# Dylan-H-Wang/skin-sm3

Measured on AMD Instinct MI355X. Metric: SM3 pretrain images/sec (paired 224x224), higher is better.
Workload: dtype bf16

## Files before the change

### skin-sm3_amd/csrc/conv_igemm.hip

```cpp
#include <stdlib.h>

#include <atomic>
#include <type_traits>

#include "conv_common.h"

using namespace sm3conv;


namespace {

#ifdef SM3_STAMP
__device__ unsigned long long* g_stamp_buf = nullptr;
__device__ long g_stamp_cap = 0;
struct StampRec {
    unsigned long long t_entry, r_entry, t_loop0 = 0, t_loop1 = 0, seg[4] = {0, 0, 0, 0}, mark[8] = {0, 0, 0, 0, 0, 0, 0, 0};
    int nsteps = 0;
    __device__ StampRec() : t_entry(__builtin_amdgcn_s_memtime()), r_entry(__builtin_amdgcn_s_memrealtime()) {}
    __device__ ~StampRec() {
        const unsigned long long t_exit = __builtin_amdgcn_s_memtime();
        const long wave = ((long)blockIdx.y * gridDim.x + blockIdx.x) * (blockDim.x / 64) + (threadIdx.x >> 6);
        if ((threadIdx.x & 63) == 0 && g_stamp_buf && wave < g_stamp_cap) {
            unsigned long long* o = g_stamp_buf + wave * 24;
            o[0] = t_entry; o[1] = t_loop0; o[2] = t_loop1; o[3] = t_exit;
            o[4] = seg[0]; o[5] = seg[1]; o[6] = seg[2]; o[7] = seg[3];
            o[8] = (unsigned long long)nsteps; o[9] = blockIdx.x; o[10] = r_entry; o[11] = __builtin_amdgcn_s_memrealtime();
            for (int i = 0; i < 8; ++i) o[12 + i] = mark[i];
            o[20] = threadIdx.x >> 6;
        }
    }
};
#define SM3_STAMP_NOW() __builtin_amdgcn_s_memtime()
#define SM3_MARK(i) (stamp.mark[i] = __builtin_amdgcn_s_memtime())
#else
#define SM3_MARK(i) ((void)0)
#endif

constexpr int kVarPw = 2, kVarNoX = 4, kVarHalo = 16, kVarGrp = 64;
template <typename T, int BM, int BN, int WM, int WN, int STAGES, int EPI, bool SEG = false, int VAR = 0>
__global__ __launch_bounds__(WM* WN * 64, (EPI >= 1 && STAGES == 1) ? 4 : 2) void conv_igemm_kernel(const ConvParams p) {
    static_assert(STAGES == 1 || STAGES == 4, "one-stage loop, or the 4-stage ring of the small-grid launches");
    constexpr bool PW = (VAR & kVarPw) != 0, NOX = (VAR & kVarNoX) != 0;
    constexpr bool HALO = (VAR & kVarHalo) != 0;
    constexpr bool GRP = (VAR & kVarGrp) != 0;
    static_assert(!GRP || (EPI == 0 && !SEG && VAR == kVarGrp), "kVarGrp: the general epilogue, one K segment");
    static_assert(!HALO || (EPI >= 1 && STAGES == 1 && !SEG && !(VAR & kVarPw) && sizeof(T) == 2 && WM * WN == 4),
                  "kVarHalo: 16-bit lean one-stage kernels, 4 waves");
    static_assert(!NOX || EPI == 3, "kVarNoX: the fused BN-backward epilogue");
#ifdef SM3_STAMP
    StampRec stamp;
#endif
    constexpr bool LEAN = EPI >= 1;
    static_assert(!(SEG && EPI == 1) && !(SEG && STAGES > 2), "segments: data-gradient epilogues, 1 or 2 stages");
    constexpr int NT = WM * WN * 64;
    constexpr int RPP = NT / 8;
    constexpr int AI = BM / RPP, BI = BN / RPP;
    constexpr int WTM = BM / WM, WTN = BN / WN, TM = WTM / 32, TN = WTN / 32;
    constexpr int SZ = sizeof(T);
    constexpr int A_BYTES = BM * 128, B_BYTES = BN * 128, STAGE = A_BYTES + B_BYTES;
    constexpr int LEAN_PITCH = BN * 2 + 16;
    constexpr int CP = BN + 4;
    constexpr int C_BYTES = LEAN ? BM * LEAN_PITCH : WTM * CP * 4;
    constexpr int MAIN_BYTES = (STAGES * STAGE > C_BYTES) ? STAGES * STAGE : C_BYTES;
    static_assert(AI >= 1 && BI >= 1 && TM >= 1 && TN >= 1, "tile too small");

    extern __shared__ __attribute__((aligned(16))) char smem[];

    const int wave = __builtin_amdgcn_readfirstlane((int)threadIdx.x >> 6);
    const int tid = (int)threadIdx.x, lane = tid & 63;
    const int wm = wave / WN, wn = wave % WN;

    int bid = blockIdx.x;
    {
        const int nwg = gridDim.x, q = nwg >> 3, r = nwg & 7, xcd = bid & 7, slot = bid >> 3;
        bid = (xcd < r ? xcd * (q + 1) : r * (q + 1) + (xcd - r) * q) + slot;
    }
    const int bn = bid % p.tilesN, bm = bid / p.tilesN;
    const int m0 = bm * BM, n0 = bn * BN;

    const long grp = GRP ? (long)blockIdx.y : 0;
    const char* const gx = GRP ? p.x + grp * p.g_x_bytes : p.x;
    const char* const gw = GRP ? p.w + grp * p.g_w_bytes : p.w;
    char* const gy = GRP ? p.y + grp * p.g_y_bytes : p.y;
    float* const gpart = (GRP && p.partials) ? p.partials + grp * p.Co : p.partials;
    const long part_ld = GRP ? (long)p.part_ld : (long)p.Co;
    const __amdgpu_buffer_rsrc_t rx = __builtin_amdgcn_make_buffer_rsrc((void*)gx, 0, p.x_bytes, 0x00020000);
    const __amdgpu_buffer_rsrc_t rw = __builtin_amdgcn_make_buffer_rsrc((void*)gw, 0, p.w_bytes, 0x00020000);
    const __amdgpu_buffer_rsrc_t rx1 =
        SEG ? __builtin_amdgcn_make_buffer_rsrc((void*)p.x1, 0, p.x1_bytes, 0x00020000) : rx;
    const __amdgpu_buffer_rsrc_t rw1 =
        SEG ? __builtin_amdgcn_make_buffer_rsrc((void*)p.w1, 0, p.w1_bytes, 0x00020000) : rw;
    const int tile_view = (p.fz_view_tiles > 0 && bm >= p.fz_view_tiles) ? 1 : 0;

    const int pos = tid & 7;
    int a_pix[AI], a_iy0[AI], a_ix0[AI];
    uint32_t a_ch[AI], a_off[AI], b_off[BI];
    uint32_t b_off1[SEG ? BI : 1];
#pragma unroll
    for (int i = 0; i < AI; ++i) {
        const int r = (tid >> 3) + i * RPP;
        a_ch[i] = (uint32_t)((pos ^ (r >> 1)) & 7) * 16u;
        const int m = m0 + r;
        if constexpr (HALO) {
            a_iy0[i] = a_ix0[i] = a_pix[i] = 0;
            continue;
        }
        if constexpr (PW) {
            a_iy0[i] = a_ix0[i] = 0;
            a_pix[i] = m < p.M ? m : -1;
            continue;
        }
        if (m < p.M) {
            const int n = fdiv(m, p.div_HoWo);
            const int rem = m - n * p.HoWo;
            const int oy = fdiv(rem, p.div_Wo);
            const int ox = rem - oy * p.Wo;
            a_iy0[i] = oy * p.sy;
            a_ix0[i] = ox * p.sx;
            a_pix[i] = (n * p.Hi + a_iy0[i]) * p.Wi + a_ix0[i];
        } else {
            a_iy0[i] = -(1 << 20);
            a_ix0[i] = 0;
            a_pix[i] = 0;
        }
    }
#pragma unroll
    for (int i = 0; i < BI; ++i) {
        const int r = (tid >> 3) + i * RPP;
        const int co = n0 + r;
        b_off[i] = (co < p.Co) ? (uint32_t)co * (uint32_t)(p.w_row_stride * SZ) + (uint32_t)((pos ^ (r >> 1)) & 7) * 16u
                               : kOOB;
        if constexpr (SEG) {
            if (co < p.Co) b_off[i] += (uint32_t)tile_view * p.w_view_bytes;
            b_off1[i] = (co < p.Co) ? (uint32_t)co * (uint32_t)(p.w1_row_stride * SZ) + (uint32_t)((pos ^ (r >> 1)) & 7) * 16u +
                                          (uint32_t)tile_view * p.w1_view_bytes
                                    : kOOB;
        }
    }
    const uint32_t row_bytes = (uint32_t)p.Ci * SZ;
    const uint32_t row_bytes1 = SEG ? (uint32_t)p.Ci1 * SZ : row_bytes;
    int cur_src = 0;

    auto set_tap = [&](int t) {
        if constexpr (SEG) cur_src = __builtin_amdgcn_readfirstlane((int)p.tap_src[t]);
        const uint32_t rb = (SEG && cur_src) ? row_bytes1 : row_bytes;
        if constexpr (PW) {
#pragma unroll
            for (int i = 0; i < AI; ++i) a_off[i] = a_pix[i] >= 0 ? (uint32_t)a_pix[i] * rb + a_ch[i] : kOOB;
            return;
        }
        const int ddy = p.dy[t], ddx = p.dx[t];
        const int dpix = ddy * p.Wi + ddx;
#pragma unroll
        for (int i = 0; i < AI; ++i) {
            const int iy = a_iy0[i] + ddy, ix = a_ix0[i] + ddx;
            const bool ok = ((unsigned)iy < (unsigned)p.Hi) && ((unsigned)ix < (unsigned)p.Wi);
            a_off[i] = ok ? (uint32_t)(a_pix[i] + dpix) * rb + a_ch[i] : kOOB;
        }
    };
    const uint32_t smem_lds = (uint32_t)(uintptr_t)((__attribute__((address_space(3))) char*)smem);
    auto dma_stage = [&](int stage, uint32_t soff_a, uint32_t soff_b) {
        const uint32_t sA = smem_lds + (uint32_t)(stage * STAGE + wave * (8 * 128));
        const uint32_t sB = sA + A_BYTES;
        if (SEG && cur_src) {
#pragma unroll
            for (int i = 0; i < AI; ++i) dma16(rx1, sA + i * (RPP * 128), a_off[i], soff_a);
#pragma unroll
            for (int i = 0; i < BI; ++i) dma16(rw1, sB + i * (RPP * 128), b_off1[SEG ? i : 0], soff_b);
            return;
        }
#pragma unroll
        for (int i = 0; i < AI; ++i) dma16(rx, sA + i * (RPP * 128), a_off[i], soff_a);
#pragma unroll
        for (int i = 0; i < BI; ++i) dma16(rw, sB + i * (RPP * 128), b_off[i], soff_b);
    };

    f32x16 acc[TM][TN];
#pragma unroll
    for (int i = 0; i < TM; ++i)
#pragma unroll
        for (int j = 0; j < TN; ++j)
#pragma unroll
            for (int r = 0; r < 16; ++r) acc[i][j][r] = 0.f;

    const int frow = lane & 31, fh = lane >> 5;
    uint32_t fa_base[TM], fb_base[TN];
#pragma unroll
    for (int i = 0; i < TM; ++i) fa_base[i] = lds_off(wm * WTM + i * 32 + frow, fh);
#pragma unroll
    for (int j = 0; j < TN; ++j) fb_base[j] = A_BYTES + lds_off(wn * WTN + j * 32 + frow, fh);

// ... 68 lines not shown
                const int n = fdiv(m, p.div_HoWo);
                const int rem = m - n * p.HoWo;
                const int oy = fdiv(rem, p.div_Wo);
                const int ox = rem - oy * p.Wo;
                const unsigned ym = (oy > 0 ? 1u : 0u) | 2u | (oy + 1 < p.Hi ? 4u : 0u);
                const unsigned xm = (ox > 0 ? 1u : 0u) | 2u | (ox + 1 < p.Wi ? 4u : 0u);
                tap_ok[i] = ((ym & 1u) ? xm : 0u) | ((ym & 2u) ? xm << 3 : 0u) | ((ym & 4u) ? xm << 6 : 0u);
            }
        }
        uint32_t fbh[TN];
#pragma unroll
        for (int j = 0; j < TN; ++j) fbh[j] = (uint32_t)p.halo_a_bytes + lds_off(wn * WTN + j * 32 + frow, fh);
        const int kchunks = p.kchunks;
#ifdef SM3_STAMP
        stamp.mark[1] = stamp.t_loop0 = SM3_STAMP_NOW();
        stamp.nsteps = 9 * kchunks;
#endif
#pragma unroll 1
        for (int c = 0; c < kchunks; ++c) {
#pragma unroll 1
            for (int tt = 0; tt < 9; ++tt) {
#ifdef SM3_STAMP
                const unsigned long long q0 = SM3_STAMP_NOW();
#endif
                if ((c | tt) != 0) __syncthreads();
#ifdef SM3_STAMP
                const unsigned long long q1 = SM3_STAMP_NOW();
#endif
                if (tt == 0) halo_issue((uint32_t)c * 128u);
                const uint32_t soff_b = (uint32_t)p.wtap[tt] * row_bytes + (uint32_t)c * 128u;
#pragma unroll
                for (int i = 0; i < BI; ++i) dma16(rw, sBw + i * (RPP * 128), b_off[i], soff_b);
                const int ddy = p.dy[tt], ddx = p.dx[tt];
                const int bit = (ddy + 1) * 3 + ddx + 1, shift = hoff + ddy * p.Wi + ddx;
                uint32_t fah[TM];
#pragma unroll
                for (int i = 0; i < TM; ++i) {
                    const uint32_t own = lds_off(frag_row[i] + shift, fh);
                    fah[i] = ((tap_ok[i] >> bit) & 1u) ? own : (uint32_t)HR * 128u + (own & 255u);
                }
#ifdef SM3_STAMP
                const unsigned long long q2 = SM3_STAMP_NOW();
#endif
                dma_drain();
#ifdef SM3_STAMP
                const unsigned long long q3 = SM3_STAMP_NOW();
#endif
                __syncthreads();
#ifdef SM3_STAMP
                const unsigned long long q4 = SM3_STAMP_NOW();
#endif
#pragma unroll
                for (int kk = 0; kk < 4; ++kk) {
                    uint4 fa[TM], fb[TN];
#pragma unroll
                    for (int i = 0; i < TM; ++i) fa[i] = *reinterpret_cast<const uint4*>(smem + (fah[i] ^ (kk << 5)));
#pragma unroll
                    for (int j = 0; j < TN; ++j) fb[j] = *reinterpret_cast<const uint4*>(smem + (fbh[j] ^ (kk << 5)));
#pragma unroll
                    for (int i = 0; i < TM; ++i)
#pragma unroll
                        for (int j = 0; j < TN; ++j) mma_frag<T>(fa[i], fb[j], acc[i][j]);
                }
#ifdef SM3_STAMP
                const unsigned long long q5 = SM3_STAMP_NOW();
                stamp.seg[0] += q2 - q1; stamp.seg[1] += q5 - q4; stamp.seg[2] += q3 - q2; stamp.seg[3] += (q1 - q0) + (q4 - q3);
#endif
            }
        }
#ifdef SM3_STAMP
        stamp.t_loop1 = SM3_STAMP_NOW();
#endif
        __syncthreads();
    } else {
    dma_stage(0, 0, wtap_off);
    if constexpr (STAGES > 2) {
        constexpr int PER = AI + BI;
        for (int s = 1; s < STAGES - 1 && s < nsteps; ++s) {
            advance();
            dma_stage(s, (uint32_t)kc * 128u, wtap_off + (uint32_t)kc * 128u);
        }
        for (int s = 0; s < nsteps; ++s) {
            const int younger = min(STAGES - 2, nsteps - 1 - s);
            if (younger >= 2) asm volatile("s_waitcnt vmcnt(%0)" ::"n"(2 * PER) : "memory");
            else if (younger == 1) asm volatile("s_waitcnt vmcnt(%0)" ::"n"(PER) : "memory");
            else dma_drain();
            __syncthreads();
            if (s + STAGES - 1 < nsteps) {
                advance();
                dma_stage((s + STAGES - 1) % STAGES, (uint32_t)kc * 128u, wtap_off + (uint32_t)kc * 128u);
            }
            compute(s % STAGES);
        }
        __syncthreads();
    } else {
        dma_drain();
        __syncthreads();
        SM3_MARK(1);
#ifdef SM3_STAMP
        stamp.nsteps = nsteps;
#endif
        for (int s = 0; s < nsteps; ++s) {
#ifdef SM3_STAMP
            const unsigned long long q0 = SM3_STAMP_NOW();
#endif
            compute(0);
#ifdef SM3_STAMP
            const unsigned long long q1 = SM3_STAMP_NOW();
#endif
            __syncthreads();
#ifdef SM3_STAMP
            const unsigned long long q2 = SM3_STAMP_NOW();
            stamp.seg[1] += q1 - q0; stamp.seg[3] += q2 - q1;
#endif
            if (s + 1 < nsteps) {
                advance();
                dma_stage(0, (uint32_t)kc * 128u, wtap_off + (uint32_t)kc * 128u);
#ifdef SM3_STAMP
                const unsigned long long q3 = SM3_STAMP_NOW();
#endif
                dma_drain();
#ifdef SM3_STAMP
                const unsigned long long q4 = SM3_STAMP_NOW();
#endif
                __syncthreads();
#ifdef SM3_STAMP
                const unsigned long long q5 = SM3_STAMP_NOW();
                stamp.seg[0] += q3 - q2; stamp.seg[2] += q4 - q3; stamp.seg[3] += q5 - q4;
#endif
            }
        }
#ifdef SM3_STAMP
        stamp.t_loop0 = stamp.mark[1];
        stamp.t_loop1 = SM3_STAMP_NOW();
#endif
    }
    }
    SM3_MARK(2);

    if constexpr (LEAN) {
        static_assert(sizeof(T) == 2, "lean epilogue is for the 16-bit types");
        constexpr int CPR = BN / 8, RSTEP = NT / CPR, NPASS = BM / RSTEP;
        char* sC = smem;
        float* sStat = reinterpret_cast<float*>(smem + (HALO ? p.halo_stat_off : MAIN_BYTES));
        const uint32_t ones = ones2<T>();
        const int cc = tid % CPR, r0 = tid / CPR;
        const int ncol = n0 + cc * 8;
        const bool fz = EPI == 3 && p.fz_partials != nullptr;
        const bool fzx = !NOX && fz && p.fz_x != nullptr;
        uint32_t eoff[EPI >= 2 ? NPASS : 1];
        uint4 pre_add[EPI >= 2 ? NPASS : 1], pre_x[(EPI == 3 && !NOX) ? NPASS : 1];
        unsigned pre_mk[EPI == 3 ? NPASS : 1];
        constexpr int NEARLY = (EPI == 3 && !NOX) ? NPASS / 2 : NPASS;
        const bool dense_out = PW || (p.osy == 1 && p.osx == 1 && p.ooy == 0 && p.oox == 0 && p.HWout == p.HoWo);
        const uint32_t pw_base = (uint32_t)(((long)(m0 + r0) * p.Co + ncol) * 2), pw_step = (uint32_t)RSTEP * (uint32_t)p.Co * 2u;
        auto request = [&](int k) {
            const int m = m0 + r0 + k * RSTEP;
            eoff[k] = ~0u;
            pre_add[k] = make_uint4(0, 0, 0, 0);
            if constexpr (EPI == 3) {
                if constexpr (!NOX) pre_x[k] = make_uint4(0, 0, 0, 0);
                pre_mk[k] = 0xffu;
            }
            if constexpr (PW) {
                if (m < p.M && ncol < p.Co) {
                    eoff[k] = pw_base + (uint32_t)k * pw_step;
                    if (p.addend) pre_add[k] = ldg16<true>(p.addend + eoff[k]);
                    if constexpr (EPI == 3) {
                        if constexpr (!NOX) {
                            if (fzx) pre_x[k] = ldg16<true>(p.fz_x + eoff[k]);
                        }
                        if (fz && p.fz_mask) pre_mk[k] = p.fz_mask[eoff[k] >> 4];
                    }
                }
                return;
            }
            if (m < p.M && ncol < p.Co) {
                long opix = m;
                int nn = 0, oy = 0, ox = 0;
                if (!dense_out || p.add_sp_h) {
                    nn = fdiv(m, p.div_HoWo);
                    const int rem = m - nn * p.HoWo;
                    oy = fdiv(rem, p.div_Wo);
                    ox = rem - oy * p.Wo;
                    if (!dense_out) opix = (long)nn * p.HWout + (long)(oy * p.osy + p.ooy) * p.Wout + (ox * p.osx + p.oox);
                }
                eoff[k] = (uint32_t)((opix * p.Co + ncol) * 2);
                if (p.addend) {
                    if (p.add_sp_h && !dense_out) {
                        pre_add[k] = ldg16<true>(p.addend + ((long)m * p.Co + ncol) * 2);
                    } else if (p.add_sp_h) {
                        if (((oy | ox) & 1) == 0)
                            pre_add[k] = ldg16<true>(p.addend + ((((long)nn * p.add_sp_h + (oy >> 1)) * p.add_sp_w + (ox >> 1)) * p.Co + ncol) * 2);
                    } else {
                        pre_add[k] = ldg16<true>(p.addend + eoff[k]);
                    }
                }
                if constexpr (EPI == 3) {
                    if constexpr (!NOX) {
                        if (fzx) pre_x[k] = ldg16<true>(p.fz_x + eoff[k]);
                    }
                    if (fz && p.fz_mask) pre_mk[k] = p.fz_mask[eoff[k] >> 4];
                }
            }
        };
        const bool epl = p.ep_scale != nullptr || p.ep_rv != nullptr;
        const bool aff = epl || (SEG && p.col_bias);
        constexpr int NCB = TN, CBW = 32;
        const int lcol = frow;
        float esc_j[NCB], esh_j[NCB];
#pragma unroll
        for (int j = 0; j < NCB; ++j) {
            esc_j[j] = 1.f;
            esh_j[j] = 0.f;
            const int gcol = n0 + wn * WTN + j * CBW + lcol;
            if (epl && gcol < p.Co) {
                if (p.ep_rv) {
                    ep_affine(p, gcol, esc_j[j], esh_j[j]);
                } else {
                    esc_j[j] = p.ep_scale[tile_view * p.Co + gcol];
                    esh_j[j] = p.ep_shift[tile_view * p.Co + gcol];
                }
            }
            if constexpr (SEG) {
                if (p.col_bias && gcol < p.Co) esh_j[j] += p.col_bias[tile_view * p.Co + gcol];
            }
        }
        if constexpr (EPI >= 2) {
#pragma unroll
            for (int k = 0; k < NEARLY; ++k) request(k);
        }
        SM3_MARK(6);
        const bool early_relu = epl && p.ep_relu && (EPI == 1 || !p.addend) && !p.ep_mask;
        auto stage_tile = [&](auto stats_c, auto aff_c, auto relu_c) {
            constexpr bool STATS = decltype(stats_c)::value, AFF = decltype(aff_c)::value, RELU = decltype(relu_c)::value;
#pragma unroll
            for (int j = 0; j < TN; ++j) {
                float s1 = 0.f, s2 = 0.f;
                char* colp = sC + (wn * WTN + j * 32 + frow) * 2 + (wm * WTM + 4 * fh) * LEAN_PITCH;
                const uint32_t colp_lds = (uint32_t)(uintptr_t)((__attribute__((address_space(3))) char*)colp);
                const float esc = esc_j[j], esh = esh_j[j];
#pragma unroll
                for (int i = 0; i < TM; ++i)
#pragma unroll
                    for (int q = 0; q < 8; ++q) {
                        float v0 = acc[i][j][2 * q], v1 = acc[i][j][2 * q + 1];
                        if constexpr (AFF) {
                            f32x2_t vv = {v0, v1};
                            vv = __builtin_elementwise_fma(vv, f32x2_t{esc, esc}, f32x2_t{esh, esh});
                            v0 = vv.x;
                            v1 = vv.y;
                            if constexpr (RELU) {
                                v0 = fmaxf(v0, 0.f);
                                v1 = fmaxf(v1, 0.f);
                            }
                        }
                        const uint32_t pk = pack2<T>(v0, v1);
                        if constexpr (STATS) {
                            s1 = dot2acc<T>(pk, ones, s1);
                            s2 = dot2acc<T>(pk, pk, s2);
                        }
                        const int R = i * 32 + (q & 1) * 2 + 8 * (q >> 1);
                        asm volatile("ds_write_b16 %0, %1 offset:%2\n\tds_write_b16_d16_hi %0, %1 offset:%3"
                                     :
                                     : "v"(colp_lds), "v"(pk), "n"(R * LEAN_PITCH), "n"((R + 1) * LEAN_PITCH)
                                     : "memory");
                    }
                if constexpr (STATS) {
                    s1 += __shfl_xor(s1, 32, 64);
                    s2 += __shfl_xor(s2, 32, 64);
                    if (lane < 32) {
                        const int col = wn * WTN + j * 32 + lane;
                        sStat[(wm * BN + col) * 2 + 0] = s1;
                        sStat[(wm * BN + col) * 2 + 1] = s2;
                    }
                }
            }
        };
        using std::true_type;
        using std::false_type;
        if (p.partials) {
            if (aff && early_relu) stage_tile(true_type{}, true_type{}, true_type{});
            else if (aff) stage_tile(true_type{}, true_type{}, false_type{});
            else stage_tile(true_type{}, false_type{}, false_type{});
        } else {
            if (aff && early_relu) stage_tile(false_type{}, true_type{}, true_type{});
            else if (aff) stage_tile(false_type{}, true_type{}, false_type{});
            else stage_tile(false_type{}, false_type{}, false_type{});
        }
        asm volatile("s_waitcnt lgkmcnt(0)" ::: "memory");
        __syncthreads();
        SM3_MARK(3);
        if (p.partials && tid < BN && n0 + tid < p.Co) {
            constexpr int G = BM / 128 > 0 ? BM / 128 : 1, WPG = WM / G;
#pragma unroll
            for (int g = 0; g < G; ++g) {
                float s1 = 0.f, s2 = 0.f;
#pragma unroll
                for (int w = 0; w < WPG; ++w) {
                    s1 += sStat[((g * WPG + w) * BN + tid) * 2 + 0];
                    s2 += sStat[((g * WPG + w) * BN + tid) * 2 + 1];
                }
                const long prow = (long)bm * G + g;
                if (G == 1 || prow * 128 < p.M) {
                    p.partials[(prow * 2 + 0) * p.Co + n0 + tid] = s1;
                    p.partials[(prow * 2 + 1) * p.Co + n0 + tid] = s2;
                }
            }
        }
        const char* sp = sC + r0 * LEAN_PITCH + cc * 16;
        if constexpr (EPI == 3) {
#pragma unroll
            for (int k = NEARLY; k < NPASS; ++k) request(k);
        }
        if constexpr (EPI == 1) {
            if (ncol < p.Co) {
                char* yp = p.y + ((long)(m0 + r0) * p.Co + ncol) * 2;
                const long ystep = (long)RSTEP * p.Co * 2;
#pragma unroll
                for (int k = 0; k < NPASS; ++k) {
                    if (m0 + r0 + k * RSTEP < p.M)
                        stg16<true>(yp + k * ystep, *reinterpret_cast<const uint4*>(sp + k * RSTEP * LEAN_PITCH));
                }
            }
            SM3_MARK(4);
            return;
        } else {
            const bool epl2 = p.ep_scale != nullptr || p.ep_rv != nullptr;
            const bool late_relu = p.ep_relu && !(epl2 && !p.addend && !p.ep_mask);
            float f_mu[8], f_is[8], f_s1[8], f_s2[8];
#pragma unroll
            for (int e = 0; e < 8; ++e) {
                f_s1[e] = f_s2[e] = f_mu[e] = f_is[e] = 0.f;
                if (EPI == 3 && fzx && ncol < p.Co) {
                    f_mu[e] = p.fz_mean[tile_view * p.Co + ncol + e];
                    f_is[e] = p.fz_invstd[tile_view * p.Co + ncol + e];
                }
            }
#pragma unroll
            for (int k = 0; k < NPASS; ++k) {
                if (eoff[k] == ~0u) continue;
                uint4 packed = *reinterpret_cast<const uint4*>(sp + k * RSTEP * LEAN_PITCH);
                if (p.addend || late_relu || (EPI == 3 && fz)) {
                    float v[8];
                    unpack16<T>(packed, v);
                    if (p.addend) {
                        float a[8];
                        unpack16<T>(pre_add[k], a);
#pragma unroll
                        for (int e = 0; e < 8; e += 2) {
                            const f32x2_t t = f32x2_t{v[e], v[e + 1]} + f32x2_t{a[e], a[e + 1]};
                            v[e] = t.x;
                            v[e + 1] = t.y;
                        }
                    }
                    if (late_relu) {
                        if (p.ep_mask) {
                            unsigned mbits = 0;
#pragma unroll
                            for (int e = 0; e < 8; ++e) mbits |= (v[e] > 0.f ? 1u : 0u) << e;
                            p.ep_mask[eoff[k] >> 4] = (uint8_t)mbits;
                        }
#pragma unroll
                        for (int e = 0; e < 8; ++e) v[e] = relu_f32(v[e]);
                    }
                    if constexpr (EPI == 3) {
                        if (fz) {
                            const unsigned mk = pre_mk[k];
#pragma unroll
                            for (int e = 0; e < 8; ++e) v[e] = keep_if_bit(v[e], mk, e);
                        }
                    }
                    packed = pack16<T>(v);
                    if constexpr (EPI == 3) {
                        if (fz) {
                            float dzr[8];
                            unpack16<T>(packed, dzr);
                            if constexpr (NOX) {
#pragma unroll
                                for (int e = 0; e < 8; ++e) f_s1[e] += dzr[e];
                            } else {
                                float xv[8];
                                unpack16<T>(pre_x[k], xv);
#pragma unroll
                                for (int e = 0; e < 8; ++e) {
                                    f_s1[e] += dzr[e];
                                    f_s2[e] += dzr[e] * (xv[e] - f_mu[e]) * f_is[e];
                                }
                            }
                        }
                    }
                }
                stg16<true>(p.y + eoff[k], packed);
            }
            SM3_MARK(4);
            if constexpr (EPI == 3) {
                if (fz) {
                    const int fz_prow = tile_view ? p.fz_row_off1 + bm - p.fz_view_tiles : p.fz_row_off + bm;
                    __syncthreads();
                    constexpr int RP = NT + 8;
                    constexpr int NSTAT = NOX ? 1 : 2;
                    float* sRed = reinterpret_cast<float*>(smem);
#pragma unroll
                    for (int e = 0; e < 8; ++e) {
                        sRed[e * RP + tid] = f_s1[e];
                        if constexpr (!NOX) sRed[(8 + e) * RP + tid] = f_s2[e];
                    }
                    __syncthreads();
                    for (int o = tid; o < 2 * BN; o += NT) {
                        const int stat = o / BN, col = o % BN;
                        float a = 0.f;
                        if (stat < NSTAT) {
                            const float* src = sRed + (stat * 8 + col % 8) * RP + col / 8;
                            for (int rl = 0; rl < NT / CPR; ++rl) a += src[rl * CPR];
                        }
                        if (n0 + col < p.Co) p.fz_partials[((long)fz_prow * 2 + stat) * p.Co + n0 + col] = a;
                    }
                    SM3_MARK(5);
                }
            }
            return;
        }
    }

    constexpr int EPC = 16 / SZ;
    constexpr int CPR = BN / EPC;
    constexpr int RSTEP = NT / CPR;
    constexpr int NROW = WTM / RSTEP;
    static_assert(NT % CPR == 0 && WTM % RSTEP == 0, "a thread must keep one channel vector across its rows");
    const bool dense = (p.osy == 1 && p.osx == 1 && p.ooy == 0 && p.oox == 0 && p.HWout == p.HoWo);
    const bool fz = p.fz_partials != nullptr;
    const bool fzx = p.fz_x != nullptr;
    const int cc = tid % CPR;
    const int ncol = n0 + cc * EPC;
    float* sC = reinterpret_cast<float*>(smem);
    float* sStat = reinterpret_cast<float*>(smem + MAIN_BYTES);

    if (p.partials) {
#pragma unroll
        for (int j = 0; j < TN; ++j) {
            float s1 = 0.f, s2 = 0.f;
#pragma unroll
            for (int i = 0; i < TM; ++i)
#pragma unroll
                for (int r = 0; r < 16; ++r) {
                    const float v = ElemTraits<T>::round(acc[i][j][r]);
                    s1 += v;
                    s2 += v * v;
                }
            s1 += __shfl_xor(s1, 32, 64);
            s2 += __shfl_xor(s2, 32, 64);
            if (lane < 32) {
                const int col = wn * WTN + j * 32 + lane;
                sStat[(wm * BN + col) * 2 + 0] = s1;
                sStat[(wm * BN + col) * 2 + 1] = s2;
            }
        }
    }

    const bool ep = p.ep_scale != nullptr || p.ep_rv != nullptr;
    const int fz_view = tile_view;
    const int fz_prow = fz_view ? p.fz_row_off1 + bm - p.fz_view_tiles : p.fz_row_off + bm;
    float f_mu[EPC], f_is[EPC], f_s1[EPC], f_s2[EPC];
#pragma unroll
    for (int e = 0; e < EPC; ++e) {
        f_s1[e] = 0.f;
        f_s2[e] = 0.f;
        f_mu[e] = 0.f;
        f_is[e] = 0.f;
        if (ncol < p.Co) {
            if (fzx) {
                f_mu[e] = p.fz_mean[fz_view * p.Co + ncol + e];
                f_is[e] = p.fz_invstd[fz_view * p.Co + ncol + e];
            } else if (ep) {
                if (p.ep_rv) {
                    ep_affine(p, ncol + e, f_is[e], f_mu[e]);
                } else {
                    f_is[e] = p.ep_scale[tile_view * p.Co + ncol + e];
                    f_mu[e] = p.ep_shift[tile_view * p.Co + ncol + e];
                }
            }
        }
    }

#pragma unroll
    for (int hh = 0; hh < WM; ++hh) {
        long e_off[NROW];
        uint4 pre_add[NROW], pre_x[NROW];
        unsigned pre_mk[NROW];
#pragma unroll
        for (int k = 0; k < NROW; ++k) {
            const int m = m0 + hh * WTM + tid / CPR + k * RSTEP;
            e_off[k] = -1;
            pre_add[k] = make_uint4(0, 0, 0, 0);
            pre_x[k] = make_uint4(0, 0, 0, 0);
            pre_mk[k] = 0xffu;
            if (m < p.M && ncol < p.Co) {
                long opix = m;
                if (!dense) {
                    const int nn = fdiv(m, p.div_HoWo);
                    const int rem = m - nn * p.HoWo;
                    const int oy = fdiv(rem, p.div_Wo);
                    const int ox = rem - oy * p.Wo;
                    opix = (long)nn * p.HWout + (long)(oy * p.osy + p.ooy) * p.Wout + (ox * p.osx + p.oox);
                }
                e_off[k] = opix * p.Co + ncol;
                if (p.addend) {
                    if (p.add_sp_h && !dense) {
                        pre_add[k] = ldg16<true>(p.addend + ((long)m * p.Co + ncol) * SZ);
                    } else if (p.add_sp_h) {
                        const int nn = fdiv(m, p.div_HoWo);
                        const int rem = m - nn * p.HoWo;
                        const int oy = fdiv(rem, p.div_Wo);
                        const int ox = rem - oy * p.Wo;
                        if (((oy | ox) & 1) == 0)
                            pre_add[k] = ldg16<true>(p.addend + ((((long)nn * p.add_sp_h + (oy >> 1)) * p.add_sp_w + (ox >> 1)) * p.Co + ncol) * SZ);
                    } else {
                        pre_add[k] = ldg16<true>(p.addend + e_off[k] * SZ);
                    }
                }
                if (fz) {
                    if (fzx) pre_x[k] = ldg16<true>(p.fz_x + e_off[k] * SZ);
                    if (p.fz_mask) pre_mk[k] = p.fz_mask[e_off[k] / EPC];
                }
            }
        }
        if (hh > 0) __syncthreads();
        if (wm == hh) {
#pragma unroll
            for (int i = 0; i < TM; ++i)
#pragma unroll
                for (int j = 0; j < TN; ++j)
#pragma unroll
                    for (int r = 0; r < 16; ++r) {
                        const int row = i * 32 + (r & 3) + 8 * (r >> 2) + 4 * fh;
                        const int col = wn * WTN + j * 32 + frow;
                        sC[row * CP + col] = acc[i][j][r];
                    }
        }
        __syncthreads();
        if (hh == 0 && p.partials && tid < BN && n0 + tid < p.Co) {
            float s1 = 0.f, s2 = 0.f;
#pragma unroll
            for (int w = 0; w < WM; ++w) {
                s1 += sStat[(w * BN + tid) * 2 + 0];
                s2 += sStat[(w * BN + tid) * 2 + 1];
// ... 13 lines not shown
                v[e + 1] = q.y;
                v[e + 2] = q.z;
                v[e + 3] = q.w;
            }
            const long boff = e_off[k] * SZ;
            if (ep) {
#pragma unroll
                for (int e = 0; e < EPC; ++e) v[e] = v[e] * f_is[e] + f_mu[e];
            }
            if constexpr (SEG) {
                if (p.col_bias) {
                    const float* cb = p.col_bias + (long)tile_view * p.Co + ncol;
#pragma unroll
                    for (int e = 0; e < EPC; ++e) v[e] += cb[e];
                }
            }
            if (p.addend) {
                float a[EPC];
                unpack16<T>(pre_add[k], a);
#pragma unroll
                for (int e = 0; e < EPC; ++e) v[e] += a[e];
            }
            if (p.ep_relu) {
                if (p.ep_mask) {
                    unsigned m = 0;
#pragma unroll
                    for (int e = 0; e < EPC; ++e) m |= (v[e] > ElemTraits<T>::kReluBit ? 1u : 0u) << e;
                    p.ep_mask[e_off[k] / EPC] = (uint8_t)m;
                }
#pragma unroll
                for (int e = 0; e < EPC; ++e) v[e] = relu_f32(v[e]);
            }
            if (fz) {
                float xv[EPC];
                unpack16<T>(pre_x[k], xv);
                const unsigned mk = pre_mk[k];
#pragma unroll
                for (int e = 0; e < EPC; ++e) v[e] = keep_if_bit(v[e], mk, e);
                const uint4 packed = pack16<T>(v);
                float dzr[EPC];
                unpack16<T>(packed, dzr);
#pragma unroll
                for (int e = 0; e < EPC; ++e) {
                    f_s1[e] += dzr[e];
                    f_s2[e] += dzr[e] * (xv[e] - f_mu[e]) * f_is[e];
                }
                stg16<true>(gy + boff, packed);
            } else {
                stg16<true>(gy + boff, pack16<T>(v));
            }
        }
    }
    if (fz) {
        __syncthreads();
        float* sRed = reinterpret_cast<float*>(smem);
#pragma unroll
        for (int e = 0; e < EPC; ++e) {
            sRed[tid * 2 * EPC + e] = f_s1[e];
            sRed[tid * 2 * EPC + EPC + e] = f_s2[e];
        }
        __syncthreads();
        for (int o = tid; o < 2 * BN; o += NT) {
            const int stat = o / BN, col = o % BN;
            float a = 0.f;
            for (int rl = 0; rl < NT / CPR; ++rl) a += sRed[(rl * CPR + col / EPC) * 2 * EPC + stat * EPC + col % EPC];
            if (n0 + col < p.Co) p.fz_partials[((long)fz_prow * 2 + stat) * p.Co + n0 + col] = a;
        }
    }
}

constexpr int kHaloLdsMax = 40960;

static int conv_halo_mode() {
    const char* v = getenv("SM3_CONV_HALO");
    return v ? atoi(v) : 1;
}
static bool conv_halo_geometry(const ConvParams& p) {
    if (!conv_halo_mode() || p.ntaps != 9 || p.x1 || p.sy != 1 || p.sx != 1 || p.add_sp_h) return false;
    const bool dense = p.osy == 1 && p.osx == 1 && p.ooy == 0 && p.oox == 0 && p.HWout == p.HoWo;
    if (!dense || p.Hi * p.Wi != p.HoWo || p.Wi != p.Wo) return false;
    unsigned seen = 0;
    for (int t = 0; t < 9; ++t) {
        if (p.dy[t] < -1 || p.dy[t] > 1 || p.dx[t] < -1 || p.dx[t] > 1) return false;
        seen |= 1u << ((p.dy[t] + 1) * 3 + p.dx[t] + 1);
    }
    return seen == 0x1ffu;
}
template <int BM, int BN>
static bool conv_halo_ok(const ConvParams& p) {
    if (!p.kord) return false;
    const int rows = BM + 2 * (p.Wi + 1) + 2;
    return ((rows + 31) / 32) * 4096 + BN * 128 <= kHaloLdsMax;
}

template <typename T, int BM, int BN, int WM, int WN, int STAGES, int EPI, bool SEG = false, int VAR = 0>
int launch_conv_st(const ConvParams& p0, hipStream_t st) {
    ConvParams p = p0;
    {
        const char* dv = getenv("SM3_CONV_DBG");
        p.dbg = dv ? atoi(dv) : 0;
    }
    constexpr bool LEAN = EPI >= 1;
    constexpr int STAGE = (BM + BN) * 128;
    constexpr int C_BYTES = LEAN ? BM * (BN * 2 + 16) : (BM / WM) * (BN + 4) * 4;
    constexpr int MAIN = (STAGES * STAGE > C_BYTES) ? STAGES * STAGE : C_BYTES;
    constexpr int STAT = WM * BN * 2 * 4;
    constexpr int LDS_STATIC = MAIN + STAT;
    static_assert(MAIN >= 256 * 2 * 8 * 4, "reduction scratch of the fused BN-backward epilogue must fit");
    int LDS = LDS_STATIC;
    if constexpr ((VAR & kVarHalo) != 0) {
        p.halo_rows = BM + 2 * (p.Wi + 1);
        p.halo_a_bytes = ((p.halo_rows + 2 + 31) / 32) * 4096;
        const int image = p.halo_a_bytes + BN * 128;
        LDS = image > C_BYTES + STAT ? image : C_BYTES + STAT;
        if (LDS > kHaloLdsMax) return SM3_EINVAL;
        p.halo_stat_off = LDS - STAT;
    }
    p.tilesM = (p.M + BM - 1) / BM;
    p.tilesN = (p.Co + BN - 1) / BN;
    auto kern = conv_igemm_kernel<T, BM, BN, WM, WN, STAGES, EPI, SEG, VAR>;
    static std::atomic<uint32_t> attr_set{0};
    int dev = 0;
    if (hipGetDevice(&dev) != hipSuccess || dev < 0 || dev > 31) dev = 0;
    if (!(attr_set.load(std::memory_order_acquire) & (1u << dev))) {
        hipError_t e = hipFuncSetAttribute(reinterpret_cast<const void*>(kern), hipFuncAttributeMaxDynamicSharedMemorySize,
                                           (VAR & kVarHalo) ? kHaloLdsMax : LDS_STATIC);
        if (e != hipSuccess) return (int)e;
        attr_set.fetch_or(1u << dev, std::memory_order_release);
    }
    const long nblocks = (long)p.tilesM * p.tilesN;
    if (nblocks <= 0 || nblocks > 0x7fffffffL) return SM3_EINVAL;
    hipLaunchKernelGGL(kern, dim3((unsigned)nblocks, (VAR & kVarGrp) ? (unsigned)p.groups : 1u), dim3(WM * WN * 64), LDS, st, p);
    SM3_CHECK_LAUNCH();
    return 0;
}

static int conv_pw_mode() {
    const char* v = getenv("SM3_CONV_PW");
    return v ? atoi(v) : 3;
}
static bool conv_is_pointwise(const ConvParams& p) {
    const bool dense = p.osy == 1 && p.osx == 1 && p.ooy == 0 && p.oox == 0 && p.HWout == p.HoWo;
    const bool taps0 = (p.x1 != nullptr) || (p.ntaps == 1 && p.dy[0] == 0 && p.dx[0] == 0);
    return dense && taps0 && p.sy == 1 && p.sx == 1 && p.Hi * p.Wi == p.HoWo && p.add_sp_h == 0;
}

template <typename T, int BM, int BN, int WM, int WN, int EPI, bool SEG>
int launch_conv_lean(const ConvParams& p, hipStream_t st) {
    if constexpr (!SEG && (EPI == 1 || EPI == 3) && WM * WN == 4) {
        if (conv_halo_ok<BM, BN>(p)) return launch_conv_st<T, BM, BN, WM, WN, 1, EPI, false, kVarHalo>(p, st);
    }
    const int mode = conv_pw_mode();
    if ((mode & 1) && conv_is_pointwise(p)) {
        if constexpr (EPI == 3 && !SEG) {
            if ((mode & 2) && p.fz_partials && !p.fz_x) return launch_conv_st<T, BM, BN, WM, WN, 1, 3, false, kVarPw | kVarNoX>(p, st);
        }
        return launch_conv_st<T, BM, BN, WM, WN, 1, EPI, SEG, kVarPw>(p, st);
    }
    return launch_conv_st<T, BM, BN, WM, WN, 1, EPI, SEG>(p, st);
}

template <typename T, int BM, int BN, int WM, int WN, int EPI>
int launch_conv_epi(const ConvParams& p, hipStream_t st, bool deep) {
    if (deep) return launch_conv_st<T, BM, BN, WM, WN, 4, EPI>(p, st);
    if constexpr (EPI >= 1 && sizeof(T) == 2) return launch_conv_lean<T, BM, BN, WM, WN, EPI, false>(p, st);
    return launch_conv_st<T, BM, BN, WM, WN, 1, EPI>(p, st);
}

template <typename T, int BM, int BN, int WM, int WN>
int launch_conv(const ConvParams& p_in, hipStream_t st) {
    ConvParams p = p_in;
    p.kord = 0;
    const char* lv = getenv("SM3_CONV_LEAN");
    const bool lean = !(lv && atoi(lv) == 0);
    if (p.x1) {
        if constexpr (sizeof(T) == 2) {
            if (lean && p.fz_partials) return launch_conv_lean<T, BM, BN, WM, WN, 3, true>(p, st);
            if (lean) return launch_conv_lean<T, BM, BN, WM, WN, 2, true>(p, st);
            return launch_conv_st<T, BM, BN, WM, WN, 1, 0, true>(p, st);
        } else {
            return SM3_EDTYPE;
        }
    }
    const long nblocks = (long)((p.M + BM - 1) / BM) * ((p.Co + BN - 1) / BN);
    const char* dv = getenv("SM3_CONV_DEEP");
    const bool deep = !(dv && atoi(dv) == 0) && nblocks <= 256 && p.ntaps * p.kchunks >= 6;
    if constexpr (sizeof(T) == 2) {
        if (lean) {
            const bool dense = p.osy == 1 && p.osx == 1 && p.ooy == 0 && p.oox == 0 && p.HWout == p.HoWo;
            p.kord = conv_halo_geometry(p) ? 1 : 0;
            if (p.fz_partials) return launch_conv_epi<T, BM, BN, WM, WN, 3>(p, st, deep);
            if (p.addend || p.ep_mask || !dense || (p.ep_scale && p.fz_view_tiles))
                return launch_conv_epi<T, BM, BN, WM, WN, 2>(p, st, deep);
            return launch_conv_epi<T, BM, BN, WM, WN, 1>(p, st, deep);
        }
    }
    return launch_conv_epi<T, BM, BN, WM, WN, 0>(p, st, deep);
}

constexpr int kBM = 128;

int fill_params(const sm3_conv_desc* d, ConvParams& p, int sz) {
    if (!d) return SM3_EINVAL;
    if (d->N <= 0 || d->Hi <= 0 || d->Wi <= 0 || d->Ci <= 0 || d->Ho <= 0 || d->Wo <= 0 || d->Co <= 0) return SM3_EINVAL;
    if (d->ntaps < 1 || d->ntaps > SM3_MAX_TAPS) return SM3_EINVAL;
    if ((d->Ci * sz) % 128 != 0) return SM3_EALIGN;
    if ((d->Co * sz) % 16 != 0) return SM3_EALIGN;
    const long M = (long)d->N * d->Ho * d->Wo;
    if (M > 0x7fffffffL) return SM3_EINVAL;
    if ((long)d->N * d->Hi * d->Wi > 0x7fffffffL) return SM3_EINVAL;
    p.M = (int)M;
    p.Hi = d->Hi; p.Wi = d->Wi; p.Ci = d->Ci; p.Co = d->Co;
    p.sy = d->sy; p.sx = d->sx; p.ntaps = d->ntaps;
    for (int t = 0; t < SM3_MAX_TAPS; ++t) { p.dy[t] = d->dy[t]; p.dx[t] = d->dx[t]; p.wtap[t] = d->wtap[t]; }
    p.w_row_stride = d->w_row_stride;
    p.Wout = d->Wout; p.HWout = d->Hout * d->Wout;
    p.osy = d->osy; p.osx = d->osx; p.ooy = d->ooy; p.oox = d->oox;
    p.HoWo = d->Ho * d->Wo; p.Wo = d->Wo;
    p.div_HoWo = make_fastdiv((uint32_t)p.HoWo);
    p.div_Wo = make_fastdiv((uint32_t)p.Wo);
    p.kchunks = d->Ci * sz / 128;
    if ((d->Ho - 1) * d->osy + d->ooy >= d->Hout || (d->Wo - 1) * d->osx + d->oox >= d->Wout) return SM3_EINVAL;
    const long xb = (long)d->N * d->Hi * d->Wi * d->Ci * sz;
    long wmax = 0;
    for (int t = 0; t < d->ntaps; ++t) wmax = d->wtap[t] > wmax ? d->wtap[t] : wmax;
    const long wb = ((long)(d->Co - 1) * d->w_row_stride + (wmax + 1) * d->Ci) * sz;
    if (xb >= 0xC0000000L || wb >= 0xC0000000L) return SM3_EINVAL;
    p.x_bytes = (uint32_t)xb;
    p.w_bytes = (uint32_t)wb;
    return 0;
}

}

extern "C" int sm3_conv_partial_rows(const sm3_conv_desc* d) {
    if (!d) return SM3_EINVAL;
    const long M = (long)d->N * d->Ho * d->Wo;
    return (int)((M + kBM - 1) / kBM);
}

struct EvalBn {
    const float *scale, *shift, *gamma, *beta, *rm, *rv;
    float eps;
    int relu;
    uint8_t* mask = nullptr;
    int views = 1;
};

static int conv_gather_gemm_impl(const sm3_conv_desc* d, const void* x, const void* w, void* y, const void* addend,
                                 float* stat_partials, const sm3_bn_bwd_fuse* fuse, void* stream,
                                 const EvalBn* ebn = nullptr, const sm3_conv_seg* seg = nullptr) {
    if (!d || !x || !w || !y) return SM3_EINVAL;
    if (fuse && ((fuse->x && (!fuse->mean || !fuse->invstd)) || !fuse->partials || fuse->partial_row_offset < 0))
        return SM3_EINVAL;
    if (!SM3_DTYPE_OK(d->dtype)) return SM3_EDTYPE;
    ConvParams p;
    const int sz = d->dtype == SM3_F32 ? 4 : 2;
    int rc = fill_params(d, p, sz);
    if (rc) return rc;
    p.x = (const char*)x; p.w = (const char*)w; p.y = (char*)y; p.addend = (const char*)addend;
    p.partials = stat_partials;
    p.fz_mask = fuse ? fuse->relu_mask : nullptr;
    p.fz_x = fuse ? (const char*)fuse->x : nullptr;
    p.fz_mean = fuse ? fuse->mean : nullptr;
    p.fz_invstd = fuse ? fuse->invstd : nullptr;
    p.fz_partials = fuse ? fuse->partials : nullptr;
    p.fz_row_off = fuse ? fuse->partial_row_offset : 0;
    p.fz_view_tiles = 0;
    p.fz_row_off1 = 0;
    p.add_sp_h = p.add_sp_w = 0;
    if (fuse && fuse->addend_sp_h > 0) {
        const bool dense = d->osy == 1 && d->osx == 1 && d->ooy == 0 && d->oox == 0 && d->Hout == d->Ho && d->Wout == d->Wo;
        const bool even_class = d->osy == 2 && d->osx == 2 && d->ooy == 0 && d->oox == 0;
        if (!addend || !(dense || even_class)) return SM3_EINVAL;
        if (dense && (fuse->addend_sp_h != (d->Ho + 1) / 2 || fuse->addend_sp_w != (d->Wo + 1) / 2)) return SM3_EINVAL;
        if (even_class && (fuse->addend_sp_h != d->Ho || fuse->addend_sp_w != d->Wo)) return SM3_EINVAL;
        p.add_sp_h = fuse->addend_sp_h;
        p.add_sp_w = fuse->addend_sp_w;
    }
    if (fuse && fuse->views > 1) {
        if (fuse->views != 2 || (p.M % 2) || ((p.M / 2) % kBM) || fuse->partial_row_offset_view1 < 0) return SM3_EALIGN;
        p.fz_view_tiles = p.M / 2 / kBM;
        p.fz_row_off1 = fuse->partial_row_offset_view1;
    }
    p.ep_scale = ebn ? ebn->scale : nullptr;
    p.ep_shift = ebn ? ebn->shift : nullptr;
    p.ep_gamma = ebn ? ebn->gamma : nullptr;
    p.ep_beta = ebn ? ebn->beta : nullptr;
    p.ep_rm = ebn ? ebn->rm : nullptr;
    p.ep_rv = ebn ? ebn->rv : nullptr;
    p.ep_eps = ebn ? ebn->eps : 0.f;
    p.ep_relu = ebn ? ebn->relu : 0;
    p.ep_mask = ebn ? ebn->mask : nullptr;
    if (ebn && ebn->views > 1) {
        if (ebn->views != 2 || fuse || (p.M % 2) || ((p.M / 2) % kBM)) return SM3_EALIGN;
        p.fz_view_tiles = p.M / 2 / kBM;
    }
    p.x1 = p.w1 = nullptr;
    p.col_bias = nullptr;
    p.x1_bytes = p.w1_bytes = p.w_view_bytes = p.w1_view_bytes = 0;
    p.Ci1 = p.kchunks1 = p.w1_row_stride = p.nsteps_seg = 0;
    for (int t = 0; t < SM3_MAX_TAPS; ++t) p.tap_src[t] = 0;
    if (seg) {
        const bool plain = d->ntaps == 1 && d->sy == 1 && d->sx == 1 && d->dy[0] == 0 && d->dx[0] == 0 && d->wtap[0] == 0 &&
                           d->osy == 1 && d->osx == 1 && d->ooy == 0 && d->oox == 0 && d->Hout == d->Ho &&
                           d->Wout == d->Wo && d->Ho == d->Hi && d->Wo == d->Wi;
        if (!plain || !seg->x1 || !seg->w1 || seg->Ci1 <= 0 || sz != 2 || (ebn && (ebn->scale || ebn->rv))) return SM3_EINVAL;
        if ((seg->Ci1 * sz) % 128 != 0) return SM3_EALIGN;
// ... 155 lines not shown
```

Before: 4649.

## Batch epilogue row stores after compute and specialize read-back on compile-time flags

Splits the lean epilogue's per-row loop into two phases. All rows are first read from LDS (with a one-ahead prefetch), transformed and stashed, and then every global store and ReLU mask byte is issued together. This is meant to remove vmcnt waits between row stores. The read-back is also instantiated on compile-time flags for addend, ReLU, mask bits and BN-stat, and the pointwise/halo paths now compute row offsets arithmetically instead of keeping per-row offsets. It also extends the pointwise NoX variant to segmented launches, and adds an asm analysis script. The cost is more template instantiations and extra register pressure from holding all rows before storing.

After: 4673, median of 6. About the same (+0.5%).

```diff
diff --git a/scratch/asm_store_waits.py b/scratch/asm_store_waits.py
--- /dev/null
+++ b/scratch/asm_store_waits.py
@@ -0,0 +1,93 @@
+import collections
+import re
+import sys
+
+src = sys.argv[1]
+want = sys.argv[2:]
+funcs, cur = collections.OrderedDict(), None
+for line in open(src):
+    m = re.match(r"^(_Z\S*conv_igemm_kernel\S*):", line)
+    if m:
+        cur = funcs.setdefault(m.group(1), {"ops": [], "mix": collections.Counter(), "vgpr": None, "scratch": None})
+        continue
+    if cur is None:
+        continue
+    s = line.strip()
+    if s.startswith("; NumVgprs:"):
+        cur["vgpr"] = int(s.split(":")[1])
+    elif s.startswith("; ScratchSize:"):
+        cur["scratch"] = int(s.split(":")[1])
+        cur = None
+        continue
+    lab = re.match(r"^(\.LBB\w+):", s)
+    if lab:
+        cur["ops"].append(("lab", lab.group(1)))
+    if not s or s[0] in ";." or s.endswith(":") or lab:
+        continue
+    op = s.split()[0]
+    kind = ("mfma" if op.startswith("v_mfma") else "valu" if op.startswith("v_") else "salu" if op.startswith("s_") else
+            "lds" if op.startswith("ds_") else "vmem" if op.startswith(("global_", "buffer_", "flat_", "scratch_")) else "other")
+    cur["mix"][kind] += 1
+    if op == "global_store_dwordx4":
+        cur["ops"].append(("ST",))
+    elif op.startswith("global_store_byte"):
+        cur["ops"].append(("sb",))
+    elif kind == "vmem":
+        cur["ops"].append(("vm",))
+    elif op == "s_waitcnt" and "vmcnt" in s:
+        cur["ops"].append(("w", int(re.search(r"vmcnt\((\d+)\)", s).group(1))))
+    elif op == "s_endpgm":
+        cur["ops"].append(("end",))
+    elif op == "s_branch" or op.startswith("s_cbranch"):
+        cur["ops"].append(("br" if op == "s_branch" else "cbr", s.split()[1]))
+
+
+def name_of(mangled):
+    m = re.search(r"kernelI(\w+?)Li(\d+)ELi(\d+)ELi(\d+)ELi(\d+)ELi(\d+)ELi(\d+)ELb([01])ELi(\d+)EEEv", mangled)
+    if not m:
+        return mangled[:60]
+    t = {"6bf16_t": "bf16", "DF16_": "f16", "f": "f32"}.get(m.group(1), m.group(1))
+    return "<%s,%s,%s,%s,%s,%s,EPI %s,SEG %s,VAR %s>" % ((t,) + m.groups()[1:])
+
+
+def analyse(ops):
+    label = {o[1]: i for i, o in enumerate(ops) if o[0] == "lab"}
+    ends = {i for i, o in enumerate(ops) if o[0] == "end"}
+    for i, o in enumerate(ops):
+        if o[0] in ("br", "cbr") and label.get(o[1], -1) > i and sum(1 for p in ops[i:label[o[1]]] if p[0] == "ST") >= 3:
+            ends.add(label[o[1]])
+    first = next((i for i, o in enumerate(ops) if o[0] == "ST"), None)
+    if first is None:
+        return ["(no 16-byte stores)"], 0
+    seq, cnt, since, pend = [], 0, -1, 0
+    for i in range(first, len(ops)):
+        o = ops[i]
+        if i in ends:
+            if seq and seq[-1] != "|":
+                seq.append("|")
+            since, pend = -1, 0
+        if o[0] == "ST":
+            since, cnt, pend = max(since, 0) + 1, cnt + pend, 0
+            seq.append("ST")
+        elif o[0] in ("sb", "vm"):
+            since = since + 1 if since >= 0 else -1
+            if o[0] == "sb":
+                seq.append("sb")
+        elif o[0] == "w":
+            flag = since >= 1 and o[1] < since
+            pend += flag
+            since = min(since, o[1]) if since >= 0 else -1
+            seq.append("%d%s" % (o[1], "!" if flag else ""))
+    return seq, cnt
+
+
+print("%-44s %5s %7s %6s %6s %5s %5s  %s" % ("instantiation <T,BM,BN,WM,WN,STAGES,EPI,SEG,VAR>", "VGPRs", "scratch", "VALU", "SALU",
+                                              "LDS", "VMEM", "stores and vmcnt waits from the first 16-byte store on"))
+for mangled, f in funcs.items():
+    name = name_of(mangled)
+    if want and not all(w in name for w in want):
+        continue
+    seq, cnt = analyse(f["ops"])
+    m = f["mix"]
+    print("%-44s %5s %7s %6d %6d %5d %5d  %s" % (name, f["vgpr"], f["scratch"], m["valu"], m["salu"], m["lds"], m["vmem"], " ".join(seq)))
+    print("%-44s vmcnt waits between two row stores: %d" % ("", cnt))
diff --git a/skin-sm3_amd/csrc/conv_igemm.hip b/skin-sm3_amd/csrc/conv_igemm.hip
--- a/skin-sm3_amd/csrc/conv_igemm.hip
+++ b/skin-sm3_amd/csrc/conv_igemm.hip
@@ -37,6 +37,11 @@
 #endif
 
 constexpr int kVarPw = 2, kVarNoX = 4, kVarHalo = 16, kVarGrp = 64;
+template <bool B>
+struct CtFlag {};
+template <bool B>
+__device__ constexpr bool flag_of(CtFlag<B>) { return B; }
+__device__ constexpr bool flag_of(bool b) { return b; }
 template <typename T, int BM, int BN, int WM, int WN, int STAGES, int EPI, bool SEG = false, int VAR = 0>
 __global__ __launch_bounds__(WM* WN * 64, (EPI >= 1 && STAGES == 1) ? 4 : 2) void conv_igemm_kernel(const ConvParams p) {
     static_assert(STAGES == 1 || STAGES == 4, "one-stage loop, or the 4-stage ring of the small-grid launches");
@@ -411,25 +416,38 @@
         uint4 pre_add[EPI >= 2 ? NPASS : 1], pre_x[(EPI == 3 && !NOX) ? NPASS : 1];
         unsigned pre_mk[EPI == 3 ? NPASS : 1];
         constexpr int NEARLY = (EPI == 3 && !NOX) ? NPASS / 2 : NPASS;
-        const bool dense_out = PW || (p.osy == 1 && p.osx == 1 && p.ooy == 0 && p.oox == 0 && p.HWout == p.HoWo);
+        constexpr bool ROWWISE = EPI == 3 && !NOX;
+        constexpr bool ROWPIX = (PW || HALO) && !ROWWISE;
+        const bool dense_out = PW || HALO || (p.osy == 1 && p.osx == 1 && p.ooy == 0 && p.oox == 0 && p.HWout == p.HoWo);
         const uint32_t pw_base = (uint32_t)(((long)(m0 + r0) * p.Co + ncol) * 2), pw_step = (uint32_t)RSTEP * (uint32_t)p.Co * 2u;
+        const int row_lim = ncol < p.Co ? p.M - m0 - r0 : 0;
+        auto row_ok = [&](int k) {
+            if constexpr (ROWPIX) return k * RSTEP < row_lim;
+            else return eoff[k] != ~0u;
+        };
+        auto row_off = [&](int k) {
+            if constexpr (ROWPIX) return pw_base + (uint32_t)k * pw_step;
+            else return eoff[k];
+        };
         auto request = [&](int k) {
             const int m = m0 + r0 + k * RSTEP;
             eoff[k] = ~0u;
             pre_add[k] = make_uint4(0, 0, 0, 0);
             if constexpr (EPI == 3) {
                 if constexpr (!NOX) pre_x[k] = make_uint4(0, 0, 0, 0);
-                pre_mk[k] = 0xffu;
-            }
-            if constexpr (PW) {
+                pre_mk[k] = 0;
+            }
+            if constexpr (PW || (HALO && !ROWWISE)) {
                 if (m < p.M && ncol < p.Co) {
-                    eoff[k] = pw_base + (uint32_t)k * pw_step;
-                    if (p.addend) pre_add[k] = ldg16<true>(p.addend + eoff[k]);
+                    const uint32_t off = pw_base + (uint32_t)k * pw_step;
+                    if constexpr (!ROWPIX) eoff[k] = off;
+                    if (p.addend) pre_add[k] = ldg16<true>(p.addend + off);
                     if constexpr (EPI == 3) {
                         if constexpr (!NOX) {
-                            if (fzx) pre_x[k] = ldg16<true>(p.fz_x + eoff[k]);
+                            if (fzx) pre_x[k] = ldg16<true>(p.fz_x + off);
                         }
-                        if (fz && p.fz_mask) pre_mk[k] = p.fz_mask[eoff[k] >> 4];
+                        pre_mk[k] = 0xffu;
+                        if (fz && p.fz_mask) pre_mk[k] = p.fz_mask[off >> 4];
                     }
                 }
                 return;
@@ -459,6 +477,7 @@
                     if constexpr (!NOX) {
                         if (fzx) pre_x[k] = ldg16<true>(p.fz_x + eoff[k]);
                     }
+                    pre_mk[k] = 0xffu;
                     if (fz && p.fz_mask) pre_mk[k] = p.fz_mask[eoff[k] >> 4];
                 }
             }
@@ -596,61 +615,153 @@
                     f_is[e] = p.fz_invstd[tile_view * p.Co + ncol + e];
                 }
             }
-#pragma unroll
-            for (int k = 0; k < NPASS; ++k) {
-                if (eoff[k] == ~0u) continue;
-                uint4 packed = *reinterpret_cast<const uint4*>(sp + k * RSTEP * LEAN_PITCH);
-                if (p.addend || late_relu || (EPI == 3 && fz)) {
-                    float v[8];
-                    unpack16<T>(packed, v);
-                    if (p.addend) {
-                        float a[8];
-                        unpack16<T>(pre_add[k], a);
-#pragma unroll
-                        for (int e = 0; e < 8; e += 2) {
-                            const f32x2_t t = f32x2_t{v[e], v[e + 1]} + f32x2_t{a[e], a[e + 1]};
-                            v[e] = t.x;
-                            v[e + 1] = t.y;
+            constexpr int NGRP = 1, GROWS = NPASS / NGRP;
+            auto read_back = [&](auto add_c, auto relu_c, auto bits_c, auto fz_c) {
+                const bool ADD = flag_of(add_c), RELU = flag_of(relu_c), BITS = flag_of(bits_c), FZ = EPI == 3 && flag_of(fz_c);
+                static_assert(NPASS <= 8, "ReLU bits of a thread's rows: two words");
+                uint32_t rb_lo = 0, rb_hi = 0;
+                uint4 next = *reinterpret_cast<const uint4*>(sp);
+#pragma unroll
+                for (int g = 0; g < NGRP; ++g) {
+#pragma unroll
+                for (int k = g * GROWS; k < (g + 1) * GROWS; ++k) {
+                    uint4 packed = next;
+                    if (k + 1 < NPASS) next = *reinterpret_cast<const uint4*>(sp + (k + 1) * RSTEP * LEAN_PITCH);
+                    if (ADD || RELU || FZ) {
+                        float v[8];
+                        unpack16<T>(packed, v);
+                        if (ADD) {
+                            float a[8];
+                            unpack16<T>(pre_add[k], a);
+#pragma unroll
+                            for (int e = 0; e < 8; e += 2) {
+                                const f32x2_t t = f32x2_t{v[e], v[e + 1]} + f32x2_t{a[e], a[e + 1]};
+                                v[e] = t.x;
+                                v[e + 1] = t.y;
+                            }
                         }
-                    }
-                    if (late_relu) {
-                        if (p.ep_mask) {
-                            unsigned mbits = 0;
-#pragma unroll
-                            for (int e = 0; e < 8; ++e) mbits |= (v[e] > 0.f ? 1u : 0u) << e;
-                            p.ep_mask[eoff[k] >> 4] = (uint8_t)mbits;
+                        if (RELU) {
+                            if (BITS) {
+                                unsigned mbits = 0;
+#pragma unroll
+                                for (int e = 0; e < 8; ++e) mbits |= (v[e] > 0.f ? 1u : 0u) << e;
+                                if (k < 4) rb_lo |= mbits << (8 * (k % 4));
+                                else rb_hi |= mbits << (8 * (k % 4));
+                                asm volatile("" : "+v"(rb_lo), "+v"(rb_hi));
+                            }
+#pragma unroll
+                            for (int e = 0; e < 8; ++e) v[e] = relu_f32(v[e]);
                         }
-#pragma unroll
-                        for (int e = 0; e < 8; ++e) v[e] = relu_f32(v[e]);
-                    }
-                    if constexpr (EPI == 3) {
-                        if (fz) {
-                            const unsigned mk = pre_mk[k];
-#pragma unroll
-                            for (int e = 0; e < 8; ++e) v[e] = keep_if_bit(v[e], mk, e);
+                        if constexpr (EPI == 3) {
+                            if (FZ) {
+                                const unsigned mk = pre_mk[k];
+#pragma unroll
+                                for (int e = 0; e < 8; ++e) v[e] = keep_if_bit(v[e], mk, e);
+                            }
                         }
-                    }
-                    packed = pack16<T>(v);
-                    if constexpr (EPI == 3) {
-                        if (fz) {
-                            float dzr[8];
-                            unpack16<T>(packed, dzr);
-                            if constexpr (NOX) {
-#pragma unroll
-                                for (int e = 0; e < 8; ++e) f_s1[e] += dzr[e];
-                            } else {
-                                float xv[8];
-                                unpack16<T>(pre_x[k], xv);
-#pragma unroll
-                                for (int e = 0; e < 8; ++e) {
-                                    f_s1[e] += dzr[e];
-                                    f_s2[e] += dzr[e] * (xv[e] - f_mu[e]) * f_is[e];
+                        packed = pack16<T>(v);
+                        if constexpr (EPI == 3) {
+                            if (FZ) {
+                                float dzr[8];
+                                unpack16<T>(packed, dzr);
+                                if constexpr (NOX) {
+#pragma unroll
+                                    for (int e = 0; e < 8; ++e) f_s1[e] += dzr[e];
+                                    asm volatile("" : "+v"(f_s1[0]), "+v"(f_s1[1]), "+v"(f_s1[2]), "+v"(f_s1[3]),
+                                                          "+v"(f_s1[4]), "+v"(f_s1[5]), "+v"(f_s1[6]), "+v"(f_s1[7]));
+                                } else {
+                                    float xv[8];
+                                    unpack16<T>(pre_x[k], xv);
+#pragma unroll
+                                    for (int e = 0; e < 8; ++e) {
+                                        f_s1[e] += dzr[e];
+                                        f_s2[e] += dzr[e] * (xv[e] - f_mu[e]) * f_is[e];
+                                    }
+                                    asm volatile("" : "+v"(f_s1[0]), "+v"(f_s1[1]), "+v"(f_s1[2]), "+v"(f_s1[3]),
+                                                          "+v"(f_s1[4]), "+v"(f_s1[5]), "+v"(f_s1[6]), "+v"(f_s1[7]),
+                                                          "+v"(f_s2[0]), "+v"(f_s2[1]), "+v"(f_s2[2]), "+v"(f_s2[3]),
+                                                          "+v"(f_s2[4]), "+v"(f_s2[5]), "+v"(f_s2[6]), "+v"(f_s2[7]));
                                 }
                             }
                         }
                     }
-                }
-                stg16<true>(p.y + eoff[k], packed);
+                    asm volatile("" : "+v"(packed.x), "+v"(packed.y), "+v"(packed.z), "+v"(packed.w));
+                    pre_add[k] = packed;
+                    __builtin_amdgcn_sched_barrier(0);
+                }
+#pragma unroll
+                for (int k = g * GROWS; k < (g + 1) * GROWS; ++k) {
+                    if (!row_ok(k)) continue;
+                    const uint32_t off = row_off(k);
+                    stg16<true>(p.y + off, pre_add[k]);
+                    if (BITS) p.ep_mask[off >> 4] = (uint8_t)((k < 4 ? rb_lo : rb_hi) >> (8 * (k % 4)));
+                }
+                }
+            };
+            const bool has_add = p.addend != nullptr, want_bits = late_relu && p.ep_mask != nullptr;
+            if constexpr (ROWWISE) {
+#pragma unroll
+                for (int k = 0; k < NPASS; ++k) {
+                    if (eoff[k] == ~0u) continue;
+                    uint4 packed = *reinterpret_cast<const uint4*>(sp + k * RSTEP * LEAN_PITCH);
+                    if (has_add || late_relu || fz) {
+                        float v[8];
+                        unpack16<T>(packed, v);
+                        if (has_add) {
+                            float a[8];
+                            unpack16<T>(pre_add[k], a);
+#pragma unroll
+                            for (int e = 0; e < 8; e += 2) {
+                                const f32x2_t t = f32x2_t{v[e], v[e + 1]} + f32x2_t{a[e], a[e + 1]};
+                                v[e] = t.x;
+                                v[e + 1] = t.y;
+                            }
+                        }
+                        if (late_relu) {
+                            if (p.ep_mask) {
+                                unsigned mbits = 0;
+#pragma unroll
+                                for (int e = 0; e < 8; ++e) mbits |= (v[e] > 0.f ? 1u : 0u) << e;
+                                p.ep_mask[eoff[k] >> 4] = (uint8_t)mbits;
+                            }
+#pragma unroll
+                            for (int e = 0; e < 8; ++e) v[e] = relu_f32(v[e]);
+                        }
+                        if (fz) {
+                            const unsigned mk = pre_mk[k];
+#pragma unroll
+                            for (int e = 0; e < 8; ++e) v[e] = keep_if_bit(v[e], mk, e);
+                        }
+                        packed = pack16<T>(v);
+                        if (fz) {
+                            float dzr[8], xv[8];
+                            unpack16<T>(packed, dzr);
+                            unpack16<T>(pre_x[NOX ? 0 : k], xv);
+#pragma unroll
+                            for (int e = 0; e < 8; ++e) {
+                                f_s1[e] += dzr[e];
+                                f_s2[e] += dzr[e] * (xv[e] - f_mu[e]) * f_is[e];
+                            }
+                        }
+                    }
+                    stg16<true>(p.y + eoff[k], packed);
+                }
+            } else if constexpr (EPI == 3) {
+                if (fz && !late_relu) {
+                    if (has_add) read_back(CtFlag<true>{}, CtFlag<false>{}, CtFlag<false>{}, CtFlag<true>{});
+                    else read_back(CtFlag<false>{}, CtFlag<false>{}, CtFlag<false>{}, CtFlag<true>{});
+                } else {
+                    read_back(has_add, late_relu, want_bits, fz);
+                }
+            } else {
+                if (late_relu == want_bits) {
+                    if (has_add && want_bits) read_back(CtFlag<true>{}, CtFlag<true>{}, CtFlag<true>{}, CtFlag<false>{});
+                    else if (want_bits) read_back(CtFlag<false>{}, CtFlag<true>{}, CtFlag<true>{}, CtFlag<false>{});
+                    else if (has_add) read_back(CtFlag<true>{}, CtFlag<false>{}, CtFlag<false>{}, CtFlag<false>{});
+                    else read_back(CtFlag<false>{}, CtFlag<false>{}, CtFlag<false>{}, CtFlag<false>{});
+                } else {
+                    read_back(has_add, true, false, false);
+                }
             }
             SM3_MARK(4);
             if constexpr (EPI == 3) {
@@ -970,8 +1081,8 @@
     }
     const int mode = conv_pw_mode();
     if ((mode & 1) && conv_is_pointwise(p)) {
-        if constexpr (EPI == 3 && !SEG) {
-            if ((mode & 2) && p.fz_partials && !p.fz_x) return launch_conv_st<T, BM, BN, WM, WN, 1, 3, false, kVarPw | kVarNoX>(p, st);
+        if constexpr (EPI == 3) {
+            if ((mode & 2) && p.fz_partials && !p.fz_x) return launch_conv_st<T, BM, BN, WM, WN, 1, 3, SEG, kVarPw | kVarNoX>(p, st);
         }
         return launch_conv_st<T, BM, BN, WM, WN, 1, EPI, SEG, kVarPw>(p, st);
     }
```
